# facebookresearch/unbiased-teacher-v2

Hardware: AMD Instinct MI355X
Metric: images/sec/node (labeled+unlabeled) UTv2 step, R50-FPN 1333x800 (higher is better)
Workload: dtype f16

## Files before the change

### include/utv2.h

```cpp
#ifndef UTV2_H
#define UTV2_H
#include <stdint.h>
#ifdef __cplusplus
extern "C" {
#endif

typedef struct ihipStream_t* utv2_stream_t;

int utv2_conv2d_nhwc_fwd(const float* x, const float* w, float* y, const float* scale, const float* bias,
                         const float* residual, int N, int H, int W, int C, int K, int KH, int KW, int stride, int pad,
                         int in_dil, int OH, int OW, int relu, int accumulate, int Kred, utv2_stream_t stream);
int utv2_conv2d_stem_fwd(const float* x, const float* w, void* y, int y_dtype, const float* scale, const float* bias, int N,
                         int H, int W, int K, int KH, int KW, int stride, int pad, int OH, int OW, int relu, int Kred,
                         utv2_stream_t stream);
int utv2_conv2d_wgrad_splits(int N, int OH, int OW, int K, int Kred);
int64_t utv2_conv2d_wgrad_workspace_floats(int N, int OH, int OW, int K, int Kred);
int utv2_conv2d_nhwc_wgrad(const float* x, const float* dy, float* dw, float* ws, int N, int H, int W, int C, int K,
                           int KH, int KW, int stride, int pad, int OH, int OW, int accumulate, utv2_stream_t stream);
int utv2_colsum(const float* g, float* db, float* ws, int M, int C, int accumulate, utv2_stream_t stream);
int utv2_weight_flip_transpose(const float* w, float* wt, int K, int KH, int KW, int C, utv2_stream_t stream);

int utv2_conv2d_ml_fwd(const float* x, const float* w, float* y, const float* scale, const float* bias,
                       const float* residual, int nlev, const int* H_host, const int* W_host, int N, int C, int K, int KH,
                       int KW, int pad, int relu, int accumulate, utv2_stream_t stream);
int utv2_conv2d_ml_wgrad(const float* x, const float* dy, float* dw, float* ws, int nlev, const int* H_host,
                         const int* W_host, int N, int C, int K, int KH, int KW, int pad, int accumulate,
                         utv2_stream_t stream);

#define UTV2_F32 0
#define UTV2_BF16 1
int utv2_conv2d_bf16_supported(int C, int KH, int KW);

int utv2_conv_clock_probe(double* ghz, double* lifetime_us);
int utv2_conv2d_nhwc_fwd_bf16(const void* x, int x_dtype, const void* w16, void* y, int y_dtype, const float* scale,
                              const float* bias, const void* residual, const void* mask, const void* post_mask, int N, int H, int W, int C, int K,
                              int KH, int KW, int stride, int pad, int in_dil, int OH, int OW, int relu, int accumulate,
                              utv2_stream_t stream);
int utv2_conv2d_nhwc_fwd_bf16_ri(const void* x, int x_dtype, const void* w16, void* y, int y_dtype, const float* scale,
                                 const float* bias, const void* residual, const void* mask, const void* post_mask, int N, int H, int W, int C,
                                 int K, int KH, int KW, int stride, int pad, int in_dil, int OH, int OW, int relu, int accumulate,
                                 const int* rowinfo, utv2_stream_t stream);
int utv2_conv2d_nhwc_fwd_bf16_bits(const void* x, int x_dtype, const void* w16, void* y, int y_dtype, const float* scale,
                                   const float* bias, const void* residual, const void* mask, const void* post_mask, int N, int H, int W,
                                   int C, int K, int KH, int KW, int stride, int pad, int in_dil, int OH, int OW, int relu, int accumulate,
                                   const int* rowinfo, void* relu_bits, const void* mask_bits, const void* post_mask_bits,
                                   utv2_stream_t stream);
int utv2_conv2d_ml_fwd_bf16(const void* x, int x_dtype, const void* w16, void* y, int y_dtype, const float* scale,
                            const float* bias, const void* residual, int nlev, const int* H_host, const int* W_host, int N,
                            int C, int K, int KH, int KW, int pad, int relu, int accumulate, utv2_stream_t stream);
int utv2_conv2d_ml_fwd_bf16_g(const void* x, int x_dtype, int x_pitch, const void* w16, void* y, int y_dtype, int y_pitch,
                              const float* scale, const float* bias, const void* residual, int nlev, const int* H_host,
                              const int* W_host, int N, int C, int K, int KH, int KW, int pad, int relu, int accumulate, int groups,
                              float* gn_part, const int* rowinfo, utv2_stream_t stream);
int utv2_conv2d_ml_fwd_bf16_gnb(const void* x, int x_pitch, const void* w16, void* y, int nlev, const int* H_host, const int* W_host, int N,
                                int C, int K, int KH, int KW, int pad, int groups, const int* rowinfo, const void* mask_bits,
                                const void* gnb_x, float* gnb_part, utv2_stream_t stream);
int utv2_conv2d_wgrad_bf16_splits(int M, int K, int Kred);
int64_t utv2_conv2d_wgrad_bf16_workspace_floats(int M, int K, int Kred);
int utv2_conv2d_wgrad_bf16(const void* x, int x_dtype, const void* dy, int dy_dtype, float* dw, float* db, float* ws,
                           const int* rowinfo, const float* rowscale, int M, int C, int K, int KH, int KW, int accumulate,
                           utv2_stream_t stream);
int utv2_conv2d_wgrad_bf16_g(const void* x, int x_dtype, int x_pitch, const void* dy, int dy_dtype, int dy_pitch, float* dw, float* db,
                             float* ws, const int* rowinfo, const float* rowscale, int M, int C, int K, int KH, int KW, int accumulate,
                             int groups, utv2_stream_t stream);
int utv2_conv2d_wgrad_bf16_d(const void* x, int x_dtype, int x_pitch, const void* dy, int dy_dtype, int dy_pitch, float* dw, float* db,
                             float* ws, const int* rowinfo, const float* rowscale, int M, int C, int K, int KH, int KW, int accumulate,
                             int groups, void* pending, utv2_stream_t stream);
int64_t utv2_wgrad_fold_table_bytes(void);
int utv2_wgrad_fold_pending(const void* pending);
int utv2_wgrad_fold_flush(void* pending, utv2_stream_t stream);
int utv2_conv2d_stem_fwd_bf16(const void* xpad16, const void* w16s, void* y, int y_dtype, const float* scale,
                              const float* bias, int N, int H, int W, int K, int OH, int OW, int relu, utv2_stream_t stream);
int utv2_rowinfo_nhwc(int* out, int N, int H, int W, int OH, int OW, int stride, int pad, int KH, int KW, int64_t start,
                      utv2_stream_t stream);
int utv2_f32_to_bf16(const float* src, void* dst16, int64_t n, utv2_stream_t stream);
int utv2_weight_flip_transpose_bf16(const float* w, void* wt16, const float* scale, int K, int KH, int KW, int C,
                                    utv2_stream_t stream);
int utv2_pad_cols_bf16(const void* src, int src_dtype, void* dst16, int64_t rows, int c, int cpad, utv2_stream_t stream);
int utv2_weight_flip_transpose_bf16_batched(const float* arena, const float* scales, void* bank, const void* table, int nlayers,
                                            utv2_stream_t stream);

int utv2_ema_axpby(float* teacher, const float* student, int64_t n, double keep_rate, utv2_stream_t stream);
int utv2_sgd_momentum(float* param, float* grad, float* mom_buf, int64_t n, float lr, float momentum, float weight_decay,
                      float grad_scale, int zero_grad, utv2_stream_t stream);
int utv2_amp_found_inf(const float* grad, int64_t n, float* state, utv2_stream_t stream);
int utv2_sgd_momentum_amp(float* param, const float* grad, float* mom_buf, int64_t n, float lr, float momentum, float weight_decay,
                          float grad_scale, const float* state, utv2_stream_t stream);
int utv2_amp_update_scale(float* state, float growth_factor, float backoff_factor, int growth_interval, utv2_stream_t stream);
int utv2_ema_axpby_m16(float* teacher, const float* student, void* mirror16, int64_t n, double keep_rate, utv2_stream_t stream);
int utv2_sgd_momentum_m16(float* param, float* grad, float* mom_buf, void* mirror16, int64_t n, float lr, float momentum, float weight_decay,
                          float grad_scale, int zero_grad, utv2_stream_t stream);
int utv2_sgd_momentum_amp_m16(float* param, const float* grad, float* mom_buf, void* mirror16, int64_t n, float lr, float momentum,
                              float weight_decay, float grad_scale, const float* state, utv2_stream_t stream);

int utv2_relu_bwd_scale(const void* dy, const void* y, const float* scale, void* out, int64_t M, int C, int dtype,
                        utv2_stream_t stream);
int utv2_add(const float* a, const float* b, float* out, int64_t n, utv2_stream_t stream);
int utv2_maxpool3x3s2_nhwc(const void* x, int x_dtype, void* y, int y_dtype, int N, int H, int W, int C, int OH, int OW,
                           utv2_stream_t stream);
int utv2_maxpool3x3s2_bwd_nhwc(const void* x, int x_dtype, const void* dpool, void* dx, int g_dtype, int N, int H, int W, int C, int OH,
                               int OW, int relu, utv2_stream_t stream);
int utv2_upsample2x_add_nhwc(const void* lateral, const void* top, void* out, int N, int H, int W, int C, int dtype,
                             utv2_stream_t stream);
int utv2_downsample2x_sum_nhwc(const void* g, void* dtop, int N, int TH, int TW, int C, int accumulate, int dtype,
                               utv2_stream_t stream);
int utv2_zero_interleave2x_nhwc(const void* src, const void* mask, void* dst, int N, int H, int W, int C, int dtype, utv2_stream_t stream);
int utv2_zero_interleave2x_add_nhwc(const void* src, const void* mask, const void* mask_bits, const void* add, void* dst, int N, int H, int W,
                                    int C, utv2_stream_t stream);
int utv2_preprocess_image(const void* src, int is_u8, float* dst, int H, int W, int Hp, int Wp,
                          const float* mean3_host, const float* std3_host, utv2_stream_t stream);
int utv2_preprocess_image_bf16pad(const void* src, int is_u8, void* dst16, int H, int W, int Hp, int Wp,
                                  const float* mean3_host, const float* std3_host, utv2_stream_t stream);
int utv2_preprocess_images_bf16pad(const void* const* src_host, int is_u8, void* dst16, const int* H_host, const int* W_host, int N,
                                   int Hp, int Wp, const float* mean3_host, const float* std3_host, utv2_stream_t stream);
int utv2_frozenbn_fold(const float* w, const float* b, const float* mean, const float* var, float* scale, float* shift,
                       int n, float eps, utv2_stream_t stream);
int64_t utv2_groupnorm_seg_workspace_floats(int nseg, const int* seg_rows_host, int C);
int utv2_groupnorm_relu_seg_fwd(const void* x, const float* gamma, const float* beta, void* y, float* mean, float* rstd,
                                float* ws, int nseg, const int* seg_rows_host, int C, int G, float eps, int relu, int dtype,
                                utv2_stream_t stream);
int utv2_groupnorm_relu_seg_fwd_p32(const void* x, const float* gamma, const float* beta, void* y, float* mean, float* rstd,
                                    const float* part32, int nseg, const int* seg_rows_host, int C, int G, float eps, int relu,
                                    utv2_stream_t stream);
int utv2_groupnorm_relu_seg_fwd_p32b(const void* x, const float* gamma, const float* beta, void* y, float* mean, float* rstd,
                                     const float* part32, int nseg, const int* seg_rows_host, int C, int G, float eps, int relu,
                                     void* relu_bits, utv2_stream_t stream);
int utv2_groupnorm_relu_seg_bwd(const void* dy, const void* y, const void* x, const float* mean, const float* rstd,
                                const float* gamma, const float* beta, void* dx, float* dgamma, float* dbeta, float* ws,
                                int nseg, const int* seg_rows_host, int C, int G, int relu, int dtype, utv2_stream_t stream);
int64_t utv2_groupnorm_seg_chunks(int nseg, const int* seg_rows_host);
int utv2_groupnorm_relu_seg_bwd_colsum(const void* dy, const void* y, const void* x, const float* mean, const float* rstd,
                                       const float* gamma, const float* beta, void* dx, float* dgamma, float* dbeta, float* ws,
                                       int nseg, const int* seg_rows_host, int C, int G, int relu, int dtype, float* colsum_part,
                                       utv2_stream_t stream);
int utv2_groupnorm_seg_bwd_p64(const void* g, const void* x, const float* mean, const float* rstd, const float* gamma, void* dx,
                               float* dgamma, float* dbeta, float* ws, int nseg, const int* seg_rows_host, int C, int G,
                               const float* part64, float* colsum_part, utv2_stream_t stream);
int utv2_colsum_partials(const float* partial, float* db, int nb, int K, int accumulate, utv2_stream_t stream);
int64_t utv2_groupnorm_workspace_floats(int N, int HW, int C);
int utv2_groupnorm_relu_fwd(const float* x, const float* gamma, const float* beta, float* y, float* mean, float* rstd,
                            float* ws, int N, int HW, int C, int G, float eps, int relu, utv2_stream_t stream);
// ... 171 lines not shown
```

### unbiased-teacher-v2_amd/csrc/conv_bf16.hip

```cpp
#include <mutex>
#include <stdlib.h>
#include "common.h"
#include <type_traits>

__device__ uint4 g_zero64[4] = {{0, 0, 0, 0}, {0, 0, 0, 0}, {0, 0, 0, 0}, {0, 0, 0, 0}};

#define CONV_MAX_LEVELS 8
struct LevelTab {
  int n;
  int start[CONV_MAX_LEVELS + 1];
  int H[CONV_MAX_LEVELS], W[CONV_MAX_LEVELS];
};

struct ConvArgs16 {
  LevelTab lt;
  const void* x;
  const h16_t* w;
  void* y;
  const float* scale;
  const float* bias;
  const void* residual;
  const void* mask;
  const void* post_mask;
  int N, H, W, C, OH, OW, K, KH, KW, stride, pad, in_dil, relu, Kred, M, accumulate;
// ... 1130 lines not shown
    int g = 0;
    for (; g + 1 < ngroups; ++g) {
      const int gb = g & 1;
      int st = g & 1;
      group_next();
      RS_SLOT_G0(0, 0, 0, true, 5) RS_SLOT_G0(1, 0, 1, true, 6)
      st ^= 1;
      RS_SLOT_G0(2, 1, 0, true, 6) RS_SLOT_G0(3, 1, 1, true, 6)
      st ^= 1;
      RS_SLOT_G0(4, 2, 0, true, 5) RS_SLOT_G0(5, 2, 1, true, 4)
    }
    {
      const int gb = g & 1;
      int st = g & 1;
      RS_SLOT_G0(0, 0, 0, false, 4) RS_SLOT_G0(1, 0, 1, false, 4)
      st ^= 1;
      load_frags(gb, 0, 1, st); prep_b(1); RS_WAIT_FRAGS; RS_BARRIER;
      compute(false, 0, 0, 0, true, st ^ 1, 1); __builtin_amdgcn_sched_barrier(0); vm_wait<4>(); RS_BARRIER;
      load_frags(gb, 1, 1, st); RS_WAIT_FRAGS; RS_BARRIER;
      compute(false, 0, 0, 0, false, 0, 0); __builtin_amdgcn_sched_barrier(0); vm_wait<2>(); RS_BARRIER;
      st ^= 1;
      load_frags(gb, 0, 2, st); RS_WAIT_FRAGS; RS_BARRIER;
      compute(false, 0, 0, 0, false, 0, 0); __builtin_amdgcn_sched_barrier(0); vm_wait<0>(); RS_BARRIER;
      load_frags(gb, 1, 2, st); RS_WAIT_FRAGS; RS_BARRIER;
      compute(false, 0, 0, 0, false, 0, 0); __builtin_amdgcn_sched_barrier(0); RS_BARRIER;
    }
    RS_BARRIER;
  } else {
    RS_BARRIER;
    int g = 0;
    for (; g + 1 < ngroups; ++g) {
      const int gb = g & 1;
      int st = g & 1;
      group_next();
      RS_SLOT_G1(0, 0, 0, true, 2) RS_SLOT_G1(1, 0, 1, true, 3)
      st ^= 1;
      RS_SLOT_G1(2, 1, 0, true, 3) RS_SLOT_G1(3, 1, 1, true, 3)
      st ^= 1;
      RS_SLOT_G1(4, 2, 0, true, 3) RS_SLOT_G1(5, 2, 1, true, 2)
    }
    {
      const int gb = g & 1;
      int st = g & 1;
      RS_SLOT_G1(0, 0, 0, false, 2) RS_SLOT_G1(1, 0, 1, false, 2)
      st ^= 1;
      load_frags(gb, 0, 1, st); prep_b(1); RS_WAIT_FRAGS; vm_wait<2>(); RS_BARRIER;
      compute(false, 0, 0, 0, true, st ^ 1, 1); __builtin_amdgcn_sched_barrier(0); RS_BARRIER;
      load_frags(gb, 1, 1, st); RS_WAIT_FRAGS; vm_wait<2>(); RS_BARRIER;
      compute(false, 0, 0, 0, false, 0, 0); __builtin_amdgcn_sched_barrier(0); RS_BARRIER;
      st ^= 1;
      load_frags(gb, 0, 2, st); RS_WAIT_FRAGS; vm_wait<0>(); RS_BARRIER;
      compute(false, 0, 0, 0, false, 0, 0); __builtin_amdgcn_sched_barrier(0); RS_BARRIER;
      load_frags(gb, 1, 2, st); RS_WAIT_FRAGS; RS_BARRIER;
      compute(false, 0, 0, 0, false, 0, 0); __builtin_amdgcn_sched_barrier(0); RS_BARRIER;
    }
  }
#undef RS_SLOT_G0
#undef RS_SLOT_G1
#undef RS_READ
#undef RS_WAIT_FRAGS
#undef RS_BARRIER
  __syncthreads();

  float* patch = (float*)smem + wid * (32 * (TN * 32 + 4));
  epilogue_rows<TN, TO, true, true, GNB>(*(const f32x16(*)[2][TN]) & acc[0], patch, lane, (TO*)p.y, p.scale, p.bias, (const TO*)p.residual,
                        p.relu, p.accumulate, m0 + wm * 128, n0 + wn * 64, p.M, p.K, (const TO*)p.mask, (const TO*)p.post_mask, p.ldy, p.gn_part, p.bits);
  epilogue_rows<TN, TO, true, true, GNB>(*(const f32x16(*)[2][TN]) & acc[2], patch, lane, (TO*)p.y, p.scale, p.bias, (const TO*)p.residual,
                        p.relu, p.accumulate, m0 + wm * 128 + 64, n0 + wn * 64, p.M, p.K, (const TO*)p.mask, (const TO*)p.post_mask, p.ldy, p.gn_part, p.bits);
  __syncthreads();
  }
  if (clk_on && threadIdx.x == 0) {
    typedef unsigned long long u64x2 __attribute__((ext_vector_type(2)));
    const u64x2 v = {__builtin_amdgcn_s_memtime() - clk_c0, __builtin_amdgcn_s_memrealtime() - clk_r0};
    *(u64x2*)g_pp_clock = v;
  }
}

static bool env_flag_on(const char* name) {
  const char* v = getenv(name);
  return !(v && v[0] == '0');
}
static const bool g_use_w8 = env_flag_on("UTV2_W8");
static const bool g_use_wgrad_w8 = env_flag_on("UTV2_WGRAD_W8");
static int env_int(const char* name, int dflt) {
  const char* v = getenv(name);
  return v ? atoi(v) : dflt;
}
static const int g_epi_general = env_int("UTV2_EPI_PLAIN", 1) ? 0 : 2;
static const int g_use_pp = env_int("UTV2_PP", 2) == 1 ? 1 : 2;

template <int BN, bool ML>
static void launch_igemm16(const ConvArgs16& a, int tiles, int x_dtype, int y_dtype, hipStream_t stream) {
  const dim3 g(tiles), b(256);
  const int64_t xelems = ML ? (int64_t)a.M * a.xs : (int64_t)a.N * a.H * a.W * a.xs;
  if (x_dtype == UTV2_BF16 && a.C % 32 == 0 && a.in_dil == 1 && a.KH * a.KW <= 16 && xelems < (1ll << 31) &&
      (int64_t)a.K * a.Kred < (1ll << 31)) {
    const bool tail = tiles > 512 && tiles <= 768;
    const bool deep = a.C % 64 == 0 && a.Kred >= 1024 && (!tail || a.bits.gnb_part);
    static const bool use_rs = env_int("UTV2_PP_RS", 1) != 0;
    const bool rs_ok = use_rs && a.rowinfo && a.KH == 3 && a.KW == 3 && a.stride == 1 && a.pad == 1 && (ML || (a.OH == a.H && a.OW == a.W));
    const bool gnb = ML && BN == 128 && a.bits.gnb_part != nullptr;
    const bool w8 = g_use_w8 && (!gnb || rs_ok);
    if (w8 && BN == 128 && a.xs >= a.groups * a.C && (a.xs & 7) == 0 && a.C % 64 == 0 && a.Kred >= 1024 && a.K >= 256 && (a.K & 3) == 0 &&
        a.m_begin == 0 && (a.groups == 1 || (a.K / a.groups) % 256 == 0)) {
      const int tilesN = cdiv(a.K, 256), tiles_m = a.M / 256, tiles_all = cdiv(a.M, 256) * tilesN;
      int main_tiles = (tiles_m * tilesN / 256) * 256;
      if (tiles_all - main_tiles > 128) main_tiles = tiles_all;
      const int main_m = main_tiles == tiles_all ? cdiv(a.M, 256) : main_tiles / tilesN;
      if (main_m > 0) {
        ConvArgs16 m = a;
        m.M = main_tiles == tiles_all ? a.M : main_m * 256;
        const int smem = 2 * (256 + 256) * 128;
        static LdsOptIn lds_opt_in;
        lds_opt_in({(const void*)conv_igemm_bf16_pp<ML, h16_t>, (const void*)conv_igemm_bf16_pp<ML, float>}, smem);
        {
          int grid = main_m * tilesN;
          static const int pp_wgs = [] { int v = env_int("UTV2_PP_WGS", 256); return v < 8 ? 8 : (v > 256 ? 256 : v / 8 * 8); }();
          if (g_use_pp == 2 && grid > 256) { m.ntiles = grid; grid = pp_wgs; }
          if (rs_ok) {
            const int smem_rs = 4 * 272 * 64 + 4 * 256 * 64 + 256;
            static LdsOptIn rs_opt_in;
            rs_opt_in({(const void*)conv_igemm_bf16_rs<ML, h16_t>, (const void*)conv_igemm_bf16_rs<ML, float>,
                       (const void*)conv_igemm_bf16_rs<ML, h16_t, ML>}, smem_rs);
            m.mtot = a.M;
            if (gnb) hipLaunchKernelGGL((conv_igemm_bf16_rs<ML, h16_t, ML>), dim3(grid), dim3(512), smem_rs, stream, m);
            else if (y_dtype == UTV2_BF16) hipLaunchKernelGGL((conv_igemm_bf16_rs<ML, h16_t>), dim3(grid), dim3(512), smem_rs, stream, m);
            else hipLaunchKernelGGL((conv_igemm_bf16_rs<ML, float>), dim3(grid), dim3(512), smem_rs, stream, m);
          } else if (y_dtype == UTV2_BF16) hipLaunchKernelGGL((conv_igemm_bf16_pp<ML, h16_t>), dim3(grid), dim3(512), smem, stream, m);
          else hipLaunchKernelGGL((conv_igemm_bf16_pp<ML, float>), dim3(grid), dim3(512), smem, stream, m);
        }
        if (m.M == a.M) return;
        ConvArgs16 r = a;
        r.m_begin = m.M;
        launch_igemm16<BN, ML>(r, cdiv(a.M - m.M, 128) * cdiv(a.K, 128), x_dtype, y_dtype, stream);
        return;
      }
    }
    if constexpr (BN == 64) {
      static const bool use_tall = env_int("UTV2_CONV_TALL64", 1) != 0;
      if (use_tall && a.KH * a.KW > 1 && a.M - a.m_begin >= 65536 && a.K > 32) {
        const dim3 gt(cdiv(a.M - a.m_begin, 256) * cdiv(a.K, 64));
        if (y_dtype == UTV2_BF16) hipLaunchKernelGGL((conv_igemm_bf16_v2<64, ML, 32, h16_t, true>), gt, b, 0, stream, a);
        else hipLaunchKernelGGL((conv_igemm_bf16_v2<64, ML, 32, float, true>), gt, b, 0, stream, a);
        return;
      }
    }
    if constexpr (BN == 96) {
      if (y_dtype == UTV2_BF16) hipLaunchKernelGGL((conv_igemm_bf16_v2<96, ML, 32, h16_t>), g, b, 0, stream, a);
      else hipLaunchKernelGGL((conv_igemm_bf16_v2<96, ML, 32, float>), g, b, 0, stream, a);
    } else if (deep) {
      if (gnb) hipLaunchKernelGGL((conv_igemm_bf16_v2<BN, ML, 64, h16_t, false, (ML && BN == 128)>), g, b, 0, stream, a);
      else if (y_dtype == UTV2_BF16) hipLaunchKernelGGL((conv_igemm_bf16_v2<BN, ML, 64, h16_t>), g, b, 0, stream, a);
      else hipLaunchKernelGGL((conv_igemm_bf16_v2<BN, ML, 64, float>), g, b, 0, stream, a);
    } else {
      if (y_dtype == UTV2_BF16) hipLaunchKernelGGL((conv_igemm_bf16_v2<BN, ML, 32, h16_t>), g, b, 0, stream, a);
      else hipLaunchKernelGGL((conv_igemm_bf16_v2<BN, ML, 32, float>), g, b, 0, stream, a);
    }
    return;
  }
  if constexpr (BN != 96) {
    if (x_dtype == UTV2_BF16) {
      if (y_dtype == UTV2_BF16) hipLaunchKernelGGL((conv_igemm_bf16<BN, ML, h16_t, h16_t>), g, b, 0, stream, a);
      else hipLaunchKernelGGL((conv_igemm_bf16<BN, ML, h16_t, float>), g, b, 0, stream, a);
    } else {
      if (y_dtype == UTV2_BF16) hipLaunchKernelGGL((conv_igemm_bf16<BN, ML, float, h16_t>), g, b, 0, stream, a);
      else hipLaunchKernelGGL((conv_igemm_bf16<BN, ML, float, float>), g, b, 0, stream, a);
// ... 592 lines not shown
      for (int j = 0; j < 2; ++j) {
        const bf16x4_t lo = __builtin_bit_cast(bf16x4_t, bl[set][j]), hi = __builtin_bit_cast(bf16x4_t, bh[set][j]);
#pragma unroll
        for (int e = 0; e < 4; ++e) { b[j][e] = lo[e]; b[j][4 + e] = hi[e]; }
      }
#pragma unroll
      for (int i = 0; i < 4; ++i)
#pragma unroll
        for (int j = 0; j < 2; ++j) {
          acc[i][j] = mfma_32x32x16(a[i], b[j], acc[i][j]);
          const int n = (set * 4 + i) * 2 + j;
          if ((n & 3) == 2) {
            __builtin_amdgcn_sched_barrier(0);
            issue_piece(stage, n >> 2);
            __builtin_amdgcn_sched_barrier(0);
          }
        }
    }
  };

  const int cb = chunk_begin;
  rload0(cb);
  rload1(cb + 1);
  WGP_VMWAIT(0);
  prep0(cb);
#pragma unroll
  for (int q = 0; q < 4; ++q) issue_piece(0, q);
  prep1(cb + 1);
#pragma unroll
  for (int q = 0; q < 4; ++q) issue_piece(1, q);
  rload0(cb + 2);
  WGP_VMWAIT(0);
  prep0(cb + 2);
#pragma unroll
  for (int q = 0; q < 4; ++q) issue_piece(2, q);
  rload1(cb + 3);
  rload0(cb + 4);
  WGP_VMWAIT(0);
  WGP_BARRIER;

  if (wm == 0) {
    for (int i = 0; i < nslots;) {
      load_slot(i & 3); prep1(cb + i + 3); WAIT_FRAGS2; WGP_BARRIER;
      rload1(cb + i + 5); compute_slot((i + 3) & 3); __builtin_amdgcn_sched_barrier(0); WGP_VMWAIT(10); WGP_BARRIER;
      if (++i >= nslots) break;
      load_slot(i & 3); prep0(cb + i + 3); WAIT_FRAGS2; WGP_BARRIER;
      rload0(cb + i + 5); compute_slot((i + 3) & 3); __builtin_amdgcn_sched_barrier(0); WGP_VMWAIT(10); WGP_BARRIER;
      ++i;
    }
    WGP_BARRIER;
  } else {
    WGP_BARRIER;
    for (int i = 0; i < nslots;) {
      WGP_VMWAIT(10); load_slot(i & 3); prep1(cb + i + 3); WAIT_FRAGS2; WGP_VMWAIT(6); WGP_BARRIER;
      rload1(cb + i + 5); compute_slot((i + 3) & 3); __builtin_amdgcn_sched_barrier(0); WGP_BARRIER;
      if (++i >= nslots) break;
      WGP_VMWAIT(10); load_slot(i & 3); prep0(cb + i + 3); WAIT_FRAGS2; WGP_VMWAIT(6); WGP_BARRIER;
      rload0(cb + i + 5); compute_slot((i + 3) & 3); __builtin_amdgcn_sched_barrier(0); WGP_BARRIER;
      ++i;
    }
  }
  WGP_VMWAIT(0);
#undef TR_READ
#undef READ_FRAGS
#undef WAIT_FRAGS2
#undef WGP_BARRIER
#undef WGP_VMWAIT

  const int frow = lane & 31, fh = lane >> 5;
  float* out = p.ws + (size_t)split * p.K * p.Kred;
#pragma unroll
  for (int j = 0; j < 2; ++j) {
    const int k = j0 + wn * 64 + j * 32 + frow;
#pragma unroll
    for (int i = 0; i < 4; ++i)
#pragma unroll
      for (int e = 0; e < 16; ++e) {
        const int co = i0 + wm * 128 + i * 32 + (e & 3) + 8 * (e >> 2) + 4 * fh;
        out[(size_t)co * p.Kred + k] = acc[i][j][e];
      }
  }
}

__global__ __launch_bounds__(256) void colsum_bf16_partial(const h16_t* __restrict__ g, float* __restrict__ partial, int M, int K,
                                                           int rows_per_block) {
  __shared__ float red[256 * 8];
  const int cpr = K >> 3;
  const int rpp = 256 / cpr;
  const int cg = threadIdx.x % cpr, rl = threadIdx.x / cpr;
  const int r0 = blockIdx.x * rows_per_block;
  int r1 = r0 + rows_per_block;
  if (r1 > M) r1 = M;
  float s[4][8];
#pragma unroll
  for (int u = 0; u < 4; ++u)
#pragma unroll
    for (int e = 0; e < 8; ++e) s[u][e] = 0.f;
  if (rl < rpp) {
    int r = r0 + rl;
    for (; r + 3 * rpp < r1; r += 4 * rpp) {
      bf16x8_t v[4];
#pragma unroll
      for (int u = 0; u < 4; ++u) v[u] = *(const bf16x8_t*)(g + (size_t)(r + u * rpp) * K + cg * 8);
#pragma unroll
      for (int u = 0; u < 4; ++u)
#pragma unroll
        for (int e = 0; e < 8; ++e) s[u][e] += (float)v[u][e];
    }
    for (; r < r1; r += rpp) {
      const bf16x8_t v = *(const bf16x8_t*)(g + (size_t)r * K + cg * 8);
#pragma unroll
      for (int e = 0; e < 8; ++e) s[0][e] += (float)v[e];
    }
  }
#pragma unroll
  for (int e = 0; e < 8; ++e) red[threadIdx.x * 8 + e] = (s[0][e] + s[1][e]) + (s[2][e] + s[3][e]);
  __syncthreads();
  for (int c = threadIdx.x; c < K; c += 256) {
    float a = 0.f;
    for (int k = 0; k < rpp; ++k) a += red[(k * cpr + (c >> 3)) * 8 + (c & 7)];
    partial[(size_t)blockIdx.x * K + c] = a;
  }
}

__global__ __launch_bounds__(256) void colsum_final_f32(const float* __restrict__ partial, float* __restrict__ db, int nb, int K,
                                                        int accumulate, const float* __restrict__ rowscale) {
  __shared__ float red[256];
  const int c = blockIdx.x * 32 + (threadIdx.x & 31), part = threadIdx.x >> 5;
  float s[4] = {0.f, 0.f, 0.f, 0.f};
  if (c < K) {
    int b = part;
    for (; b + 24 < nb; b += 32) {
#pragma unroll
      for (int u = 0; u < 4; ++u) s[u] += partial[(size_t)(b + 8 * u) * K + c];
    }
    for (; b < nb; b += 8) s[0] += partial[(size_t)b * K + c];
  }
  red[threadIdx.x] = (s[0] + s[1]) + (s[2] + s[3]);
  __syncthreads();
  if (part == 0 && c < K) {
    float v = 0.f;
#pragma unroll
    for (int k = 0; k < 8; ++k) v += red[threadIdx.x + 32 * k];
    if (rowscale) v *= rowscale[c];
    db[c] = accumulate ? db[c] + v : v;
  }
}

__global__ __launch_bounds__(256) void reduce_slabs16_f32(const float* __restrict__ ws, float* __restrict__ dst, size_t n, int splits,
                                                          int accumulate, const float* __restrict__ rowscale, int rowlen) {
  const size_t n4 = n >> 2;
  size_t i = (size_t)blockIdx.x * blockDim.x + threadIdx.x;
  const size_t stride = (size_t)gridDim.x * blockDim.x;
  for (; i < n4; i += stride) {
    f32x4 s[4];
#pragma unroll
    for (int u = 0; u < 4; ++u) s[u] = f32x4{0.f, 0.f, 0.f, 0.f};
    int k = 0;
    for (; k + 4 <= splits; k += 4) {
#pragma unroll
      for (int u = 0; u < 4; ++u) s[u] += ((const f32x4*)(ws + (size_t)(k + u) * n))[i];
    }
    for (; k < splits; ++k) s[0] += ((const f32x4*)(ws + (size_t)k * n))[i];
    f32x4 t = (s[0] + s[1]) + (s[2] + s[3]);
    if (rowscale) {
      const float r = rowscale[(i * 4) / rowlen];
// ... 65 lines not shown
      if (f.rowscale) s *= f.rowscale[i];
      f.dst[i] = f.accumulate ? f.dst[i] + s : s;
    }
  } else {
    const int K = (int)f.n, nb = f.splits;
    const int c = lb * 32 + (threadIdx.x & 31), part = threadIdx.x >> 5;
    float s[4] = {0.f, 0.f, 0.f, 0.f};
    if (c < K) {
      int b = part;
      for (; b + 24 < nb; b += 32) {
#pragma unroll
        for (int u = 0; u < 4; ++u) s[u] += f.ws[(size_t)(b + 8 * u) * K + c];
      }
      for (; b < nb; b += 8) s[0] += f.ws[(size_t)b * K + c];
    }
    red[threadIdx.x] = (s[0] + s[1]) + (s[2] + s[3]);
    __syncthreads();
    if (part == 0 && c < K) {
      float v = 0.f;
#pragma unroll
      for (int k = 0; k < 8; ++k) v += red[threadIdx.x + 32 * k];
      if (f.rowscale) v *= f.rowscale[c];
      f.dst[c] = f.accumulate ? f.dst[c] + v : v;
    }
  }
}

static int slab_fold_add(SlabFoldTable* t, int kind, const float* ws, float* dst, const float* rowscale, size_t n, int splits, int accumulate,
                         int rowlen) {
  if (t->count < 0 || t->count >= SLAB_FOLD_MAX) return UTV2_EARG;
  for (int i = 0; i < t->count; ++i)
    if (t->e[i].dst == dst) return UTV2_EARG;
  SlabFold& f = t->e[t->count];
  f.kind = kind; f.ws = ws; f.dst = dst; f.rowscale = rowscale; f.n = n; f.splits = splits; f.accumulate = accumulate; f.rowlen = rowlen;
  int nb;
  if (kind == 0) { nb = cdiv((int64_t)n / 4, 256); if (nb > 2048) nb = 2048; }
  else if (kind == 1) nb = cdiv((int64_t)n, 256);
  else nb = cdiv((int64_t)n, 32);
  if (nb < 1) nb = 1;
  f.blk0 = t->count == 0 ? 0 : t->e[t->count - 1].blk0 + t->e[t->count - 1].nblk;
  f.nblk = nb;
  t->total_blocks = f.blk0 + nb;
  ++t->count;
  return UTV2_OK;
}

extern "C" {

static int wgrad16_small_splits(int M, int K, int Kred) {
  const int chunks = cdiv(M, 32);
  const int tiles = cdiv(K, 128) * cdiv(Kred, 128);
  const double flop = 2.0 * M * K * Kred;
  int splits = cdiv(flop > 512 * 2.0e8 ? 1024 : 512, tiles);
  const int max_by_chunks = chunks / 8 > 0 ? chunks / 8 : 1;
  if (splits > max_by_chunks) splits = max_by_chunks;
  if (splits < 1) splits = 1;
  if (splits > 256) splits = 256;
  if (splits >= 8) splits = (splits + 7) / 8 * 8 <= max_by_chunks ? (splits + 7) / 8 * 8 : splits / 8 * 8;
  return splits;
}

#define WGRAD_W8_MAX_NB 1024
static int wgrad16_w8_budget() {
  static const int w = [] {
    int v = env_int("UTV2_WGRAD_W8_WGS", 256);
    v = (v / 8) * 8;
    return v < 8 ? 8 : (v > 256 ? 256 : v);
  }();
  return w;
}
static int wgrad16_w8_splits(int M, int K, int Kred) {
  const int tiles = (K >> 8) * (Kred >> 8), chunks = cdiv(M, WGRAD_W8_BP);
  int splits = wgrad16_w8_budget() / tiles;
  if (splits > chunks / 8) splits = chunks / 8;
  return splits < 1 ? 1 : splits;
}
static bool wgrad16_w8_shape_ok(int M, int C, int K, int KH, int KW, int xs, int groups) {
  const int Kred = KH * KW * C, tiles = (K >> 8) * (Kred >> 8), chunks = cdiv(M, WGRAD_W8_BP);
  if ((K & 255) || (C & 255) || KH * KW > 16 || K > 2048 || tiles > wgrad16_w8_budget() || chunks < 16 || (int64_t)M * K >= (1ll << 31) ||
      (int64_t)M * xs >= (1ll << 31) || (xs & 7) || ((K / groups) & 255))
    return false;
  if (KH * KW == 1 && chunks < 16 * (256 / tiles)) return false;
  return true;
}

int utv2_conv2d_wgrad_bf16_splits(int M, int K, int Kred) { return wgrad16_small_splits(M, K, Kred); }

int utv2_colsum_partials(const float* partial, float* db, int nb, int K, int accumulate, hipStream_t stream) {
  if (!partial || !db || nb < 1 || K < 1) return UTV2_EARG;
  hipLaunchKernelGGL(colsum_final_f32, dim3(cdiv(K, 32)), dim3(256), 0, stream, partial, db, nb, K, accumulate, (const float*)nullptr);
  return utv2_launch_status();
}

int64_t utv2_conv2d_wgrad_bf16_workspace_floats(int M, int K, int Kred) {
  int64_t n = (int64_t)wgrad16_small_splits(M, K, Kred) * ((int64_t)K * Kred + K);
  if ((K & 255) == 0 && (Kred & 255) == 0) {
    const int64_t n8 = (int64_t)wgrad16_w8_splits(M, K, Kred) * K * Kred + (int64_t)WGRAD_W8_MAX_NB * K;
    if (n8 > n) n = n8;
  }
  return n;
}

static int wgrad_bf16_impl(const void* x, int x_dtype, int x_pitch, const void* dy, int dy_dtype, int dy_pitch, float* dw, float* db,
                           float* ws, const int* rowinfo, const float* rowscale, int M, int C, int K, int KH, int KW, int accumulate,
                           int groups, hipStream_t stream, SlabFoldTable* pending = nullptr);

int utv2_conv2d_wgrad_bf16(const void* x, int x_dtype, const void* dy, int dy_dtype, float* dw, float* db, float* ws,
                           const int* rowinfo, const float* rowscale, int M, int C, int K, int KH, int KW, int accumulate,
                           hipStream_t stream) {
  return wgrad_bf16_impl(x, x_dtype, C, dy, dy_dtype, K, dw, db, ws, rowinfo, rowscale, M, C, K, KH, KW, accumulate, 1, stream);
}

int utv2_conv2d_wgrad_bf16_g(const void* x, int x_dtype, int x_pitch, const void* dy, int dy_dtype, int dy_pitch, float* dw, float* db,
                             float* ws, const int* rowinfo, const float* rowscale, int M, int C, int K, int KH, int KW, int accumulate,
                             int groups, hipStream_t stream) {
  return wgrad_bf16_impl(x, x_dtype, x_pitch, dy, dy_dtype, dy_pitch, dw, db, ws, rowinfo, rowscale, M, C, K, KH, KW, accumulate, groups,
                         stream);
}

int utv2_conv2d_wgrad_bf16_d(const void* x, int x_dtype, int x_pitch, const void* dy, int dy_dtype, int dy_pitch, float* dw, float* db,
                             float* ws, const int* rowinfo, const float* rowscale, int M, int C, int K, int KH, int KW, int accumulate,
                             int groups, void* pending, hipStream_t stream) {
  if (!pending) return UTV2_EARG;
  SlabFoldTable* t = (SlabFoldTable*)pending;
  if (t->count < 0 || t->count + 3 > SLAB_FOLD_MAX) return UTV2_EARG;
  return wgrad_bf16_impl(x, x_dtype, x_pitch, dy, dy_dtype, dy_pitch, dw, db, ws, rowinfo, rowscale, M, C, K, KH, KW, accumulate, groups,
                         stream, t);
}

int64_t utv2_wgrad_fold_table_bytes(void) { return (int64_t)sizeof(SlabFoldTable); }

int utv2_wgrad_fold_pending(const void* pending) { return pending ? ((const SlabFoldTable*)pending)->count : -1; }

int utv2_wgrad_fold_flush(void* pending, hipStream_t stream) {
  if (!pending) return UTV2_EARG;
  SlabFoldTable* t = (SlabFoldTable*)pending;
  if (t->count < 0 || t->count > SLAB_FOLD_MAX) return UTV2_EARG;
  if (t->count == 0) return UTV2_OK;
  hipLaunchKernelGGL(reduce_slabs_table, dim3(t->total_blocks), dim3(256), 0, stream, *t);
  t->count = 0;
  t->total_blocks = 0;
  return utv2_launch_status();
}

static int wgrad_bf16_impl(const void* x, int x_dtype, int x_pitch, const void* dy, int dy_dtype, int dy_pitch, float* dw, float* db,
                           float* ws, const int* rowinfo, const float* rowscale, int M, int C, int K, int KH, int KW, int accumulate,
                           int groups, hipStream_t stream, SlabFoldTable* pending) {
  if (!x || !dy || !dw || !ws || !rowinfo || (C & 7) || (K & 7) || M <= 0 || KH * KW > 16 || bad_dtype(x_dtype) ||
      bad_dtype(dy_dtype) || groups < 1 || K % groups || x_pitch < groups * C || (groups > 1 && (K / groups) % 128) ||
      (x_pitch != C && (x_pitch & (x_dtype == UTV2_BF16 ? 7 : 3))) || dy_pitch < K || (dy_pitch != K && (dy_pitch & (dy_dtype == UTV2_BF16 ? 7 : 3))))
    return UTV2_EARG;
  Wgrad16Args a;
  a.x = x; a.dy = dy; a.ws = ws; a.rowinfo = (const int2*)rowinfo;
  a.C = C; a.K = K; a.KH = KH; a.KW = KW; a.Kred = KH * KW * C; a.M = M; a.debug = 0; a.xs = x_pitch; a.groups = groups; a.dys = dy_pitch;
  if (g_use_wgrad_w8 && x_dtype == UTV2_BF16 && dy_dtype == UTV2_BF16 && dy_pitch == K && wgrad16_w8_shape_ok(M, C, K, KH, KW, x_pitch, groups)) {
    a.splits = wgrad16_w8_splits(M, K, a.Kred);
    a.chunks_per_split = cdiv(cdiv(M, WGRAD_W8_BP), a.splits);
    a.bias_ws = nullptr;
    const size_t n = (size_t)K * a.Kred;
    const int smem = 2 * 2 * WGRAD_W8_BP * 512;
    static LdsOptIn pp_opt_in;
    pp_opt_in({(const void*)conv_wgrad_bf16_pp}, smem);
    hipLaunchKernelGGL(conv_wgrad_bf16_pp, dim3(wgrad16_w8_budget()), dim3(512), smem, stream, a);
    int rb = cdiv((int64_t)n / 4, 256);
    if (rb > 8192) rb = 8192;
    if (pending) {
      if (int rc = slab_fold_add(pending, 0, ws, dw, rowscale, n, a.splits, accumulate, a.Kred)) return rc;
    } else
      hipLaunchKernelGGL(reduce_slabs16_f32, dim3(rb), dim3(256), 0, stream, (const float*)ws, dw, n, a.splits, accumulate, rowscale,
                         a.Kred);
    if (db) {
      float* part = ws + (size_t)a.splits * n;
      int nb = cdiv(M, 64);
      if (nb > WGRAD_W8_MAX_NB) nb = WGRAD_W8_MAX_NB;
      const int rows = cdiv(M, nb);
      nb = cdiv(M, rows);
      hipLaunchKernelGGL(colsum_bf16_partial, dim3(nb), dim3(256), 0, stream, (const h16_t*)dy, part, M, K, rows);
      if (pending) {
        if (int rc = slab_fold_add(pending, 2, part, db, rowscale, (size_t)K, nb, accumulate, 1)) return rc;
      } else
        hipLaunchKernelGGL(colsum_final_f32, dim3(cdiv(K, 32)), dim3(256), 0, stream, (const float*)part, db, nb, K, accumulate, rowscale);
    }
    return utv2_launch_status();
  }
  a.splits = utv2_conv2d_wgrad_bf16_splits(M, K, a.Kred);
  a.chunks_per_split = cdiv(cdiv(M, 32), a.splits);
  const size_t n = (size_t)K * a.Kred;
  a.bias_ws = db ? ws + (size_t)a.splits * n : nullptr;
  const int tiles = cdiv(K, 128) * cdiv(a.Kred, 128);
  const dim3 g(tiles * a.splits), b(256);
  if (x_dtype == UTV2_BF16) {
    if (dy_dtype == UTV2_BF16) hipLaunchKernelGGL((conv_wgrad_bf16<h16_t, h16_t>), g, b, 0, stream, a);
    else hipLaunchKernelGGL((conv_wgrad_bf16<h16_t, float>), g, b, 0, stream, a);
  } else {
    if (dy_dtype == UTV2_BF16) hipLaunchKernelGGL((conv_wgrad_bf16<float, h16_t>), g, b, 0, stream, a);
    else hipLaunchKernelGGL((conv_wgrad_bf16<float, float>), g, b, 0, stream, a);
  }
  int rb = cdiv((int64_t)n / 4, 256);
  if (rb > 8192) rb = 8192;
  if (pending) {
    if (int rc = slab_fold_add(pending, 0, ws, dw, rowscale, n, a.splits, accumulate, a.Kred)) return rc;
    if (db)
      if (int rc = slab_fold_add(pending, 1, a.bias_ws, db, rowscale, (size_t)K, a.splits, accumulate, 1)) return rc;
    return utv2_launch_status();
  }
  hipLaunchKernelGGL(reduce_slabs16_f32, dim3(rb), dim3(256), 0, stream, (const float*)ws, dw, n, a.splits, accumulate, rowscale,
                       a.Kred);
  if (db)
    hipLaunchKernelGGL(reduce_slabs16_scalar_f32, dim3(cdiv(K, 256)), dim3(256), 0, stream, (const float*)a.bias_ws, db, (size_t)K,
                       a.splits, accumulate, rowscale);
  return utv2_launch_status();
}

}
```

Measured before the change: 343.5.

## Add DMA-pipelined bf16 wgrad kernel for 1x1 convs without bias

Adds a new weight-gradient kernel for 1x1 convolutions. It streams dy and x rows straight into LDS through global_load_lds in a 4-stage ring buffer, then reads the fragments back with transposing LDS reads to feed 32x32 MFMAs. Row-info prefetch and the next stage's loads are interleaved with the MFMAs, to hide global memory latency that the register-staged kernel exposes. It is enabled by default through an env flag, covers bf16 x/dy 1x1 shapes with no bias gradient, and adds a routing query to the header. Risks are correctness of the hand-tuned waitcnt counts and extra LDS use that may lower occupancy.

```diff
diff --git a/include/utv2.h b/include/utv2.h
--- a/include/utv2.h
+++ b/include/utv2.h
@@ -57,6 +57,7 @@
                                 const void* gnb_x, float* gnb_part, utv2_stream_t stream);
 int utv2_conv2d_wgrad_bf16_splits(int M, int K, int Kred);
 int64_t utv2_conv2d_wgrad_bf16_workspace_floats(int M, int K, int Kred);
+int utv2_wgrad_bf16_route(int M, int C, int K, int KH, int KW, int x_pitch, int dy_pitch, int groups, int has_db);
 int utv2_conv2d_wgrad_bf16(const void* x, int x_dtype, const void* dy, int dy_dtype, float* dw, float* db, float* ws,
                            const int* rowinfo, const float* rowscale, int M, int C, int K, int KH, int KW, int accumulate,
                            utv2_stream_t stream);
diff --git a/unbiased-teacher-v2_amd/csrc/conv_bf16.hip b/unbiased-teacher-v2_amd/csrc/conv_bf16.hip
--- a/unbiased-teacher-v2_amd/csrc/conv_bf16.hip
+++ b/unbiased-teacher-v2_amd/csrc/conv_bf16.hip
@@ -1236,6 +1236,7 @@
 }
 static const bool g_use_w8 = env_flag_on("UTV2_W8");
 static const bool g_use_wgrad_w8 = env_flag_on("UTV2_WGRAD_W8");
+static const bool g_use_wgrad_dma = env_flag_on("UTV2_WGRAD_DMA");
 static int env_int(const char* name, int dflt) {
   const char* v = getenv(name);
   return v ? atoi(v) : dflt;
@@ -1994,6 +1995,211 @@
   }
 }
 
+template <int NS>
+__global__ __launch_bounds__(256) void conv_wgrad_bf16_dma(Wgrad16Args p) {
+  constexpr int BP = 32, ROWB = 256, OPB = BP * ROWB, STAGE = 2 * OPB;
+  static_assert(NS == 3 || NS == 4, "ring depth");
+  __shared__ __attribute__((aligned(16))) unsigned char smem[NS * STAGE];
+  const int tid = threadIdx.x, lane = tid & 63;
+  const int wid = __builtin_amdgcn_readfirstlane(tid >> 6);
+  const int wm = wid >> 1, wn = wid & 1;
+  const int tilesN = (p.Kred + 127) / 128, tilesM = (p.K + 127) / 128;
+  const int tiles = tilesM * tilesN;
+  int split, bid;
+  if ((p.splits & 7) == 0) {
+    const int xcd = blockIdx.x & 7, idx = blockIdx.x >> 3;
+    split = xcd + 8 * (idx / tiles);
+    bid = idx % tiles;
+  } else {
+    split = blockIdx.x / tiles;
+    bid = blockIdx.x - split * tiles;
+  }
+  const int mt = bid / tilesN, nt = bid - mt * tilesN;
+  const int i0 = mt * 128, j0 = nt * 128;
+  const int goff = p.groups > 1 ? (i0 / (p.K / p.groups)) * p.C : 0;
+
+  f32x16 acc[2][2];
+#pragma unroll
+  for (int i = 0; i < 2; ++i)
+#pragma unroll
+    for (int j = 0; j < 2; ++j)
+#pragma unroll
+      for (int e = 0; e < 16; ++e) acc[i][j][e] = 0.f;
+
+  const int total_chunks = (p.M + BP - 1) / BP;
+  const int cb = split * p.chunks_per_split;
+  int chunk_end = cb + p.chunks_per_split;
+  if (chunk_end > total_chunks) chunk_end = total_chunks;
+  const int nslots = chunk_end - cb;
+
+  const int hr = lane >> 4, ps = lane & 15;
+  const int choff = (((ps >> 2) ^ hr) << 5) + ((ps & 3) << 3);
+  const int co8 = i0 + choff;
+  const bool aok = co8 < p.K;
+  const int kk = j0 + choff;
+  const bool bok = kk < p.Kred;
+  const int tap = bok ? kk / p.C : 0;
+  const int ci = (bok ? kk - tap * p.C : 0) + goff;
+  const int dh = tap / p.KW, dw = tap - dh * p.KW;
+  const int rowl = 8 * wid + hr;
+  const h16_t* xl = (const h16_t*)p.x + ci;
+  const h16_t* dyl = (const h16_t*)p.dy + co8;
+  const h16_t* zero = (const h16_t*)g_zero64;
+  typedef int i32x2 __attribute__((ext_vector_type(2)));
+  i32x2 ri[2][2];
+  const h16_t* psrc[4];
+  auto rload = [&](int chunk, i32x2 (&r)[2]) {
+#pragma unroll
+    for (int q = 0; q < 2; ++q) {
+      int m = chunk * BP + rowl + 4 * q;
+      m = m < p.M ? m : p.M - 1;
+      const int2* src = p.rowinfo + m;
+      asm volatile("global_load_dwordx2 %0, %1, off" : "=v"(r[q]) : "v"(src));
+    }
+  };
+  auto prep = [&](int chunk, const i32x2 (&r)[2]) {
+#pragma unroll
+    for (int q = 0; q < 2; ++q) {
+      const int m = chunk * BP + rowl + 4 * q;
+      const bool in = (m < p.M) & (chunk < chunk_end);
+      const bool oka = in & aok;
+      psrc[q] = (oka ? dyl : zero) + (size_t)(unsigned)(oka ? m : 0) * (unsigned)p.dys;
+      const int W = r[q].y >> 16;
+      const bool okb = in & bok & (bool)((r[q].y >> tap) & 1);
+      psrc[2 + q] = (okb ? xl : zero) + (size_t)(unsigned)(okb ? r[q].x + dh * W + dw : 0) * (unsigned)p.xs;
+    }
+  };
+  auto issue_piece = [&](int stage, int q4) {
+    unsigned char* dst = smem + stage * STAGE + (q4 < 2 ? 0 : OPB) + (8 * wid + 4 * (q4 & 1)) * ROWB;
+    __builtin_amdgcn_global_load_lds((gptr_t)psrc[q4], (lptr_t)dst, 16, 0, 0);
+  };
+
+  const int G = lane >> 4, t = lane & 15, r3 = t >> 2;
+  const unsigned lbase = (unsigned)(size_t)(lptr_t)smem;
+  const unsigned lrow = lbase + (8 * (G >> 1) + r3) * ROWB + 32 * (G & 1) + 8 * (t & 3);
+  unsigned aoff[2], boff[2];
+#pragma unroll
+  for (int i = 0; i < 2; ++i) {
+    aoff[i] = lrow + (((wm * 2 + i) ^ r3) << 6);
+    boff[i] = OPB + lrow + (((wn * 2 + i) ^ r3) << 6);
+  }
+
+  typedef short s16x4 __attribute__((ext_vector_type(4)));
+  s16x4 al[2][2], ah[2][2], bl[2][2], bh[2][2];
+#define TR_READ(dst, addr, off) asm volatile("ds_read_b64_tr_b16 %0, %1 offset:%2" : "=v"(dst) : "v"(addr), "n"(off))
+#define READ_FRAGS(S)                                                                          \
+  TR_READ(al[S][0], ab[0], (S) * 16 * ROWB); TR_READ(ah[S][0], ab[0], ((S) * 16 + 4) * ROWB);  \
+  TR_READ(al[S][1], ab[1], (S) * 16 * ROWB); TR_READ(ah[S][1], ab[1], ((S) * 16 + 4) * ROWB);  \
+  TR_READ(bl[S][0], bb[0], (S) * 16 * ROWB); TR_READ(bh[S][0], bb[0], ((S) * 16 + 4) * ROWB);  \
+  TR_READ(bl[S][1], bb[1], (S) * 16 * ROWB); TR_READ(bh[S][1], bb[1], ((S) * 16 + 4) * ROWB)
+#define WAIT_FRAGS(N, S)                                                                                               \
+  asm volatile("s_waitcnt lgkmcnt(" #N ")"                                                                              \
+               : "+v"(al[S][0]), "+v"(al[S][1]), "+v"(ah[S][0]), "+v"(ah[S][1]), "+v"(bl[S][0]), "+v"(bl[S][1]), "+v"(bh[S][0]), \
+                 "+v"(bh[S][1]))
+#define WGD_VMWAIT(N) asm volatile("s_waitcnt vmcnt(" #N ")" : "+v"(ri[0][0]), "+v"(ri[0][1]), "+v"(ri[1][0]), "+v"(ri[1][1]) : : "memory")
+#define WGD_BARRIER                         \
+  __builtin_amdgcn_sched_barrier(0);        \
+  __builtin_amdgcn_s_barrier();             \
+  __builtin_amdgcn_sched_barrier(0)
+
+  auto slot = [&](int i, int st, i32x2 (&r)[2]) {
+    if constexpr (NS == 4) { WGD_VMWAIT(10); } else { WGD_VMWAIT(6); }
+    prep(cb + i + NS - 1, r);
+    WGD_BARRIER;
+    rload(cb + i + NS + 1, r);
+    unsigned ab[2], bb[2];
+#pragma unroll
+    for (int k = 0; k < 2; ++k) {
+      ab[k] = aoff[k] + st * STAGE;
+      bb[k] = boff[k] + st * STAGE;
+    }
+    READ_FRAGS(0);
+    READ_FRAGS(1);
+    const int sp = st == 0 ? NS - 1 : st - 1;
+#pragma unroll
+    for (int s = 0; s < 2; ++s) {
+      if (s == 0) { WAIT_FRAGS(8, 0); } else { WAIT_FRAGS(0, 1); }
+      bf16x8_t a[2], b[2];
+#pragma unroll
+      for (int k = 0; k < 2; ++k) {
+        const bf16x4_t alo = __builtin_bit_cast(bf16x4_t, al[s][k]), ahi = __builtin_bit_cast(bf16x4_t, ah[s][k]);
+        const bf16x4_t blo = __builtin_bit_cast(bf16x4_t, bl[s][k]), bhi = __builtin_bit_cast(bf16x4_t, bh[s][k]);
+#pragma unroll
+        for (int e = 0; e < 4; ++e) {
+          a[k][e] = alo[e]; a[k][4 + e] = ahi[e];
+          b[k][e] = blo[e]; b[k][4 + e] = bhi[e];
+        }
+      }
+#pragma unroll
+      for (int ii = 0; ii < 2; ++ii)
+#pragma unroll
+        for (int j = 0; j < 2; ++j) {
+          acc[ii][j] = mfma_32x32x16(a[ii], b[j], acc[ii][j]);
+          if (j == 1) {
+            __builtin_amdgcn_sched_barrier(0);
+            issue_piece(sp, s * 2 + ii);
+            __builtin_amdgcn_sched_barrier(0);
+          }
+        }
+    }
+  };
+
+  if (nslots > 0) {
+    rload(cb, ri[0]);
+    rload(cb + 1, ri[1]);
+    WGD_VMWAIT(0);
+    prep(cb, ri[0]);
+#pragma unroll
+    for (int q = 0; q < 4; ++q) issue_piece(0, q);
+    prep(cb + 1, ri[1]);
+#pragma unroll
+    for (int q = 0; q < 4; ++q) issue_piece(1, q);
+    if constexpr (NS == 4) {
+      rload(cb + 2, ri[0]);
+      WGD_VMWAIT(0);
+      prep(cb + 2, ri[0]);
+#pragma unroll
+      for (int q = 0; q < 4; ++q) issue_piece(2, q);
+      rload(cb + 3, ri[1]);
+      rload(cb + 4, ri[0]);
+    } else {
+      rload(cb + 2, ri[0]);
+      rload(cb + 3, ri[1]);
+    }
+    WGD_VMWAIT(0);
+    int st = 0;
+    for (int i = 0; i < nslots;) {
+      if constexpr (NS == 4) slot(i, st, ri[1]); else slot(i, st, ri[0]);
+      st = st + 1 == NS ? 0 : st + 1;
+      if (++i >= nslots) break;
+      if constexpr (NS == 4) slot(i, st, ri[0]); else slot(i, st, ri[1]);
+      st = st + 1 == NS ? 0 : st + 1;
+      ++i;
+    }
+    WGD_VMWAIT(0);
+  }
+#undef TR_READ
+#undef READ_FRAGS
+#undef WAIT_FRAGS
+#undef WGD_VMWAIT
+#undef WGD_BARRIER
+
+  const int frow = lane & 31, fh = lane >> 5;
+  float* out = p.ws + (size_t)split * p.K * p.Kred;
+#pragma unroll
+  for (int j = 0; j < 2; ++j) {
+    const int k = j0 + wn * 64 + j * 32 + frow;
+    if (k >= p.Kred) continue;
+#pragma unroll
+    for (int i = 0; i < 2; ++i)
+#pragma unroll
+      for (int e = 0; e < 16; ++e) {
+        const int co = i0 + wm * 64 + i * 32 + (e & 3) + 8 * (e >> 2) + 4 * fh;
+        if (co < p.K) out[(size_t)co * p.Kred + k] = acc[i][j][e];
+      }
+  }
+}
+
 __global__ __launch_bounds__(256) void colsum_bf16_partial(const h16_t* __restrict__ g, float* __restrict__ partial, int M, int K,
                                                            int rows_per_block) {
   __shared__ float red[256 * 8];
@@ -2225,6 +2431,14 @@
     return false;
   if (KH * KW == 1 && chunks < 16 * (256 / tiles)) return false;
   return true;
+}
+
+static bool wgrad16_dma_shape_ok(int K, int Kred, int KH, int KW, bool has_db) {
+  return g_use_wgrad_dma && KH * KW == 1 && !has_db && cdiv(K, 128) * cdiv(Kred, 128) >= 4;
+}
+int utv2_wgrad_bf16_route(int M, int C, int K, int KH, int KW, int x_pitch, int dy_pitch, int groups, int has_db) {
+  if (g_use_wgrad_w8 && dy_pitch == K && wgrad16_w8_shape_ok(M, C, K, KH, KW, x_pitch, groups)) return 2;
+  return wgrad16_dma_shape_ok(K, KH * KW * C, KH, KW, has_db != 0) ? 1 : 0;
 }
 
 int utv2_conv2d_wgrad_bf16_splits(int M, int K, int Kred) { return wgrad16_small_splits(M, K, Kred); }
@@ -2333,8 +2547,10 @@
   const int tiles = cdiv(K, 128) * cdiv(a.Kred, 128);
   const dim3 g(tiles * a.splits), b(256);
   if (x_dtype == UTV2_BF16) {
-    if (dy_dtype == UTV2_BF16) hipLaunchKernelGGL((conv_wgrad_bf16<h16_t, h16_t>), g, b, 0, stream, a);
-    else hipLaunchKernelGGL((conv_wgrad_bf16<h16_t, float>), g, b, 0, stream, a);
+    if (dy_dtype == UTV2_BF16) {
+      if (wgrad16_dma_shape_ok(K, a.Kred, KH, KW, db != nullptr)) hipLaunchKernelGGL(conv_wgrad_bf16_dma<4>, g, b, 0, stream, a);
+      else hipLaunchKernelGGL((conv_wgrad_bf16<h16_t, h16_t>), g, b, 0, stream, a);
+    } else hipLaunchKernelGGL((conv_wgrad_bf16<h16_t, float>), g, b, 0, stream, a);
   } else {
     if (dy_dtype == UTV2_BF16) hipLaunchKernelGGL((conv_wgrad_bf16<float, h16_t>), g, b, 0, stream, a);
     else hipLaunchKernelGGL((conv_wgrad_bf16<float, float>), g, b, 0, stream, a);
```

Result: no change. 345.1 (median of 6 runs) (+0.5%).
